# Elyptos/VolumetricRaytracer

Measured on AMD Instinct MI355X. Metric: Mrays/sec at 1080p, 256^3 SDF volume, higher is better.
Workload: dtype f32

## Files before the change

### volumetricraytracer_amd/csrc/vrt_device.h

```cpp
#pragma once
#include <stdint.h>

namespace vrt {

constexpr int kBrickCells = 4;
constexpr int kBrickSamples = 5;
constexpr int kBrickFloats = 128;
constexpr int kPathCube = 8;
constexpr int kPathBrick16 = 9;
constexpr int kPathCube16 = 10;
constexpr int kPathCells16 = 11;
constexpr int kNibWindow = 16;
constexpr int kTile = 8;
constexpr int kBlockThreads = 256;
constexpr int kMaxBvhNodes = 2 * 64 - 1;
constexpr int kStatWords = 7;
constexpr int kStatRecord = 8;
constexpr int kDiagRecord = 8;
constexpr int kMaxBlocks = 1 << 20;
#ifndef VRT_MAX_BLOCK_FRAMES
#define VRT_MAX_BLOCK_FRAMES 48
#endif
constexpr int kMaxBlockFrames = VRT_MAX_BLOCK_FRAMES;
constexpr int kMaxLaunchFrames = 256;

constexpr int kMapSupertile = 0;
constexpr int kMapBand = 1;
constexpr int kMapLinear = 2;

inline int grid_blocks(int tiles_x, int tiles_y, int tile_map) {
    if (tile_map != kMapSupertile) return tiles_x * tiles_y;
    const int st = ((tiles_x + 3) / 4) * ((tiles_y + 3) / 4);
    return ((st + 7) / 8) * 8 * 16;
}

struct DVolume {
    const float* dense;
    const void* bricks;
    const void* cells;
    int32_t N;
    int32_t nb;
    float extent;
    float inv_cell;
    float density_scale;
    float step_max;
    float tint[3];
    float roughness;
    float metallic;
    float k;
    float cell;
    int32_t format;
    const uint8_t* skip;
    const uint32_t* nib;
    const uint8_t* tex_px[3];
    int32_t tex_w[3], tex_h[3];
    float tex_scale[2];
// ... 133 lines not shown
```

### volumetricraytracer_amd/csrc/vrt_kernels.hip

```cpp
#include <hip/hip_runtime.h>
#include <math.h>
#include <stdlib.h>
#include "vrt_device.h"
#include "vrt_launch.h"
#include "voxelize_core.h"
#include "brush_core.h"

namespace vrt {

struct F3 {
    float x, y, z;
};
__device__ __forceinline__ F3 f3(float x, float y, float z) { return F3{x, y, z}; }
__device__ __forceinline__ F3 operator+(F3 a, F3 b) { return f3(a.x + b.x, a.y + b.y, a.z + b.z); }
__device__ __forceinline__ F3 operator-(F3 a, F3 b) { return f3(a.x - b.x, a.y - b.y, a.z - b.z); }
__device__ __forceinline__ F3 operator*(F3 a, float s) { return f3(a.x * s, a.y * s, a.z * s); }
__device__ __forceinline__ float dot3(F3 a, F3 b) { return (a.x * b.x + a.y * b.y) + a.z * b.z; }
__device__ __forceinline__ F3 normalize3(F3 a) {
    float inv = 1.0f / sqrtf(dot3(a, a));
    return a * inv;
}
__device__ __forceinline__ float maxf_(float a, float b) { return a > b ? a : b; }
__device__ __forceinline__ float minf_(float a, float b) { return a < b ? a : b; }
__device__ __forceinline__ F3 mul33(const float* m, F3 v) {
// ... 694 lines not shown
        return march_cube<NORMAL, PATH == kPathCube16>(F, I, Vd, o, d, t_cur, t_hit, n_world, steps, ex);
    } else {
    constexpr int DP = data_path<PATH>();
    const VolRef V = load_vol<DP>(Vd);
    RaySeg R;
    if constexpr (DIR_SHADOW) {
        if (!setup_shadow_ray(F, I, V, o, t_cur, t_base, R)) return false;
    } else {
        if (!setup_ray(F, I, V, o, d, t_cur, t_base, R)) return false;
    }
    MarchState st;
    st.t = st.t_prev = R.t0;
    st.s_prev = st.s_hit = 0.0f;
    st.i = 0;
    st.hit = false;
    st.chk = __builtin_inff();
    st.c = Cell{0, 0, 0, 0.0f, 0.0f, 0.0f};
    march_lane<DP, DIAG, MULTI>(F, V, R, st, F.max_steps, steps, dg);
    if (!st.hit) {
        if (F.max_steps > 0 && st.i >= F.max_steps && !(st.t > R.t_end)) ex += kExhaustedOne;
        return false;
    }
    float t = st.t;
    Cell c = st.c;
    if (st.s_hit < 0.0f && st.i > 0) t = refine_hit<DP>(V, R, st.t_prev, st.s_prev, t, st.s_hit, c, steps);
    else if (NORMAL != 0 && F.polish > 0 && st.i > 0) t = polish_hit<DP>(F, V, R, t, st.s_hit, st.t_prev, st.s_prev, F.polish, c, steps);
    t_hit = t;
    if constexpr (NORMAL == 1) n_world = hit_normal<DP, false, REF>(I, V, R, c, st.i, REF && F.zero_outside != 0);
    if constexpr (NORMAL == 2) n_world = hit_normal<DP, true, REF>(I, V, R, c, st.i, REF && F.zero_outside != 0);
    return true;
    }
}

template <int PATH, bool SINGLE, bool DIAG = false, int NORMAL = 1, bool REF = false>
__device__ __forceinline__ bool trace_closest(const DFrame& F, F3 o, F3 d, float t_max, float t_base, float& t_best,
                                              int& inst_best, F3& n_best, unsigned& steps, unsigned& ex, DiagAcc* dg = nullptr) {
    if constexpr (SINGLE) {
        float t;
        F3 n;
        if (march_instance<PATH, NORMAL, DIAG, false, REF>(F, F.inst, F.vol0, o, d, t_max, t_base, t, n, steps, ex, dg)) {
            t_best = t;
            inst_best = 0;
            n_best = n;
            return true;
        }
        return false;
    } else {
        bool any = false;
        float best = t_max;
        int ni = 0;
        while (ni < F.n_nodes) {
            ni = __builtin_amdgcn_readfirstlane(ni);
            const DBvhNode nd = F.nodes[ni];
            const bool in = slab_box(o, d, nd, best);
            if (__ballot(in) == 0ull) {
                ni = nd.right;
                continue;
            }
            if (nd.left < 0) {
                const int ii = -nd.left - 1;
                const DInstance* I = F.inst + ii;
                if (in) {
                    float t;
                    F3 n;
                    constexpr bool kCube = PATH == kPathCube || PATH == kPathCube16;
                    if (march_instance<PATH, NORMAL, DIAG, false, REF, true>(F, I, F.vols + I->slot, o, d, kCube ? best : t_max, t_base, t, n, steps, ex, dg)) {
                        if (!any || t < best || (t == best && ii < inst_best)) {
                            any = true;
                            best = t;
                            t_best = t;
                            inst_best = ii;
                            n_best = n;
                        }
                    }
                }
                ni = nd.right;
            } else {
                ni = ni + 1;
            }
        }
        return any;
    }
}

template <int PATH, bool SINGLE, bool DIAG = false, bool DIR_SHADOW = false>
__device__ __forceinline__ bool trace_any(const DFrame& F, F3 o, F3 d, float t_max, float t_base, unsigned& steps, unsigned& ex,
                                          DiagAcc* dg = nullptr) {
    float t;
    F3 n;
    if constexpr (SINGLE) {
        return march_instance<PATH, 0, DIAG, DIR_SHADOW>(F, F.inst, F.vol0, o, d, t_max, t_base, t, n, steps, ex, dg);
    } else {
        bool found = false;
        int ni = 0;
        while (ni < F.n_nodes) {
            if (__ballot(!found) == 0ull) break;
            ni = __builtin_amdgcn_readfirstlane(ni);
            const DBvhNode nd = F.nodes[ni];
            const bool in = !found && slab_box(o, d, nd, t_max);
            if (__ballot(in) == 0ull) {
                ni = nd.right;
                continue;
            }
            if (nd.left < 0) {
                const DInstance* I = F.inst + (-nd.left - 1);
                if (in && march_instance<PATH, 0, DIAG, DIR_SHADOW, false, true>(F, I, F.vols + I->slot, o, d, t_max, t_base, t, n, steps, ex, dg)) found = true;
                ni = nd.right;
            } else {
                ni = ni + 1;
            }
        }
        return found;
    }
}

__device__ __forceinline__ unsigned env_fetch(const uint8_t* __restrict__ env, int S, F3 dir) {
    if (env == nullptr) return 0u;
    float vx = dir.x, vy = dir.z, vz = dir.y;
    float ax = fabsf(vx), ay = fabsf(vy), az = fabsf(vz);
    int face;
    float sc, tc, ma;
    if (ax >= ay && ax >= az) {
        ma = ax;
        if (vx >= 0.0f) { face = 0; sc = -vz; tc = -vy; }
        else            { face = 1; sc = vz;  tc = -vy; }
    } else if (ay >= az) {
        ma = ay;
        if (vy >= 0.0f) { face = 2; sc = vx; tc = vz; }
        else            { face = 3; sc = vx; tc = -vz; }
    } else {
        ma = az;
        if (vz >= 0.0f) { face = 4; sc = vx;  tc = -vy; }
        else            { face = 5; sc = -vx; tc = -vy; }
    }
    const float inv_ma = 1.0f / ma;
    float u = (sc * inv_ma + 1.0f) * 0.5f;
    float v = (tc * inv_ma + 1.0f) * 0.5f;
    int ix = (int)floorf(u * (float)S);
    int iy = (int)floorf(v * (float)S);
// ... 22 lines not shown
    float m = maxf_(-wdoth + 1.0f, 0.0f);
    float m2 = m * m;
    float m5 = (m2 * m2) * m;
    F3 Fr = f3(f0.x + (-f0.x + 1.0f) * m5, f0.y + (-f0.y + 1.0f) * m5, f0.z + (-f0.z + 1.0f) * m5);
    float dwo = maxf_(dot3(n, wo), 0.0f);
    float dwi = maxf_(dot3(n, wi), 0.0f);
    float G = (dwo * fast_rcp(dwo * (1.0f - k) + k)) * (dwi * fast_rcp(dwi * (1.0f - k) + k));
    float dg = (D * G) * fast_rcp(maxf_((4.0f * dwo) * dwi, 0.0001f));
    F3 cook = f3(dg * Fr.x, dg * Fr.y, dg * Fr.z);
    float km = 1.0f - metal;
    F3 kd = f3((1.0f - Fr.x) * km, (1.0f - Fr.y) * km, (1.0f - Fr.z) * km);
    return f3((albedo.x * INV_PI_REF) * kd.x + cook.x * Fr.x, (albedo.y * INV_PI_REF) * kd.y + cook.y * Fr.y,
              (albedo.z * INV_PI_REF) * kd.z + cook.z * Fr.z);
}

__device__ __forceinline__ F3 radiance(F3 Li, F3 wi, F3 wo, F3 n, F3 albedo, float rough, float metal, float k) {
    const F3 brdf = brdf_eval(wi, wo, n, albedo, rough, metal, k);
    const float ndwi = dot3(n, wi);
    return f3((brdf.x * Li.x) * ndwi, (brdf.y * Li.y) * ndwi, (brdf.z * Li.z) * ndwi);
}

__device__ __forceinline__ float tonemap(float c) {
    c = c > 0.0f ? c : 0.0f;
    c = c * fast_rcp(c + 1.0f);
    return fast_pow(c, 1.0f / 2.2f);
}

__device__ __forceinline__ unsigned wave_sum(unsigned v) {
#pragma unroll
    for (int o = 32; o > 0; o >>= 1) v += __shfl_xor(v, o);
    return v;
}

__device__ __forceinline__ void tile_of_block(const DFrame& F, int b, int nblk, int& tile_x, int& tile_y) {
    if (F.tile_map == kMapSupertile) {
        const int rot = (int)blockIdx.y;
        const int xcd = (b + rot) & 7, q = b >> 3;
        const int st = (q >> 4) * 8 + xcd;
        const int within = q & 15;
        const int st_x = (F.tiles_x + 3) >> 2;
        tile_x = (st % st_x) * 4 + (within & 3);
        tile_y = (st / st_x) * 4 + (within >> 2);
    } else if (F.tile_map == kMapBand) {
        const int xcd = b & 7, q = b >> 3;
        const int per = nblk >> 3, rem = nblk & 7;
        const int L = (xcd < rem) ? xcd * (per + 1) + q : rem * (per + 1) + (xcd - rem) * per + q;
        tile_x = L % F.tiles_x;
        tile_y = L / F.tiles_x;
    } else {
        tile_x = b % F.tiles_x;
        tile_y = b / F.tiles_x;
    }
}

constexpr int kMarchThreads = 64;
constexpr int kMarchGridMul = 4;
__device__ __forceinline__ void block_and_wave(int& b, int& wave) {
    const int raw = (int)blockIdx.x, xcd = raw & 7, q = raw >> 3;
    wave = q & 3;
    b = ((q >> 2) << 3) | xcd;
}

__device__ __forceinline__ void pixel_of_lane(int tile_x, int tile_y, int wave, int lane, int& px, int& pyl) {
    px = tile_x * 16 + (wave & 1) * 8 + (lane & 7);
    pyl = tile_y * 16 + (wave >> 1) * 8 + (lane >> 3);
}

__device__ __forceinline__ bool wave_can_reach(const DCam& C, bool valid, int px, int py) {
    const int x0 = (int)(C.cull_lo & 0xffffu), y0 = (int)(C.cull_lo >> 16), x1 = (int)(C.cull_hi & 0xffffu), y1 = (int)(C.cull_hi >> 16);
    const bool inside = px >= x0 && px <= x1 && py >= y0 && py <= y1;
    return __ballot(valid && inside) != 0ull;
}

__device__ __forceinline__ DCam load_cam(const DBlock& B, int frame) {
    typedef unsigned u16v __attribute__((ext_vector_type(16)));
    u16v w;
    if (B.f.cams != nullptr) w = *reinterpret_cast<const u16v __attribute__((address_space(4)))*>((const __attribute__((address_space(4))) DCam*)B.f.cams + frame);
    else w = *reinterpret_cast<const u16v*>(&B.cam[frame]);
    DCam C;
    C.cam_o[0] = __uint_as_float(w[0]); C.cam_o[1] = __uint_as_float(w[1]); C.cam_o[2] = __uint_as_float(w[2]);
    C.r0[0] = __uint_as_float(w[3]); C.r0[1] = __uint_as_float(w[4]); C.r0[2] = __uint_as_float(w[5]);
    C.r1[0] = __uint_as_float(w[6]); C.r1[1] = __uint_as_float(w[7]); C.r1[2] = __uint_as_float(w[8]);
    C.r2[0] = __uint_as_float(w[9]); C.r2[1] = __uint_as_float(w[10]); C.r2[2] = __uint_as_float(w[11]);
    C.cx = __uint_as_float(w[12]); C.cy = __uint_as_float(w[13]);
    C.cull_lo = w[14]; C.cull_hi = w[15];
    return C;
}

template <bool DYN>
__device__ __forceinline__ const DFrame& frame_view(const DBlock& B, int frame, DFrame& Fd) {
    if constexpr (!DYN) {
        (void)frame;
        (void)Fd;
        return B.f;
    } else {
        typedef unsigned u16v __attribute__((ext_vector_type(16)));
        Fd = B.f;
        const char* sec = static_cast<const char*>(B.f.dyn) + (size_t)(unsigned)frame * kDynStride;
        const u16v w = *reinterpret_cast<const u16v __attribute__((address_space(4)))*>((const __attribute__((address_space(4))) char*)sec);
        Fd.light_dir[0] = __uint_as_float(w[0]);
        Fd.light_dir[1] = __uint_as_float(w[1]);
        Fd.light_dir[2] = __uint_as_float(w[2]);
        Fd.light_strength = __uint_as_float(w[3]);
        Fd.n_inst = (int)w[4];
        Fd.n_nodes = (int)w[5];
        Fd.n_point = (int)w[6];
        Fd.n_spot = (int)w[7];
        Fd.vol0 = B.f.vols + (int)w[8];
        Fd.inst = reinterpret_cast<const DInstance*>(sec + kDynInstOff);
        Fd.nodes = reinterpret_cast<const DBvhNode*>(sec + kDynNodesOff);
        Fd.point = reinterpret_cast<const DPointLight*>(sec + kDynPointOff);
        Fd.spot = reinterpret_cast<const DSpotLight*>(sec + kDynSpotOff);
        return Fd;
    }
}

__device__ __forceinline__ void camera_ray(const DFrame& F, const DCam& C, int px, int py, F3& o, F3& d) {
    float sx = (((float)px + 0.5f) * F.inv_w) * 2.0f - 1.0f;
    float sy = (((float)py + 0.5f) * F.inv_h) * 2.0f - 1.0f;
// ... 202 lines not shown
    return q;
}
__device__ __forceinline__ F3 rotate_vector(F3 v, Q4 r) {
    Q4 rc = {-r.x, -r.y, -r.z, r.w};
    Q4 vq = {v.x, v.y, v.z, 0.0f};
    const Q4 t = qmul(r, qmul(vq, rc));
    return f3(t.x, t.y, t.z);
}

template <bool CONST_ONLY = false>
__device__ __forceinline__ void textured_surface(const DVolume* __restrict__ V, const DInstance* __restrict__ I, F3 hit_world,
                                                 F3& albedo, F3& n, float& rough, float& metal) {
    const F3 op = mul33(I->w2o, f3(hit_world.x - I->pos[0], hit_world.y - I->pos[1], hit_world.z - I->pos[2]));
    const F3 no = mul33(I->w2o, n);
    const F3 an = f3(fabsf(no.x), fabsf(no.y), fabsf(no.z));
    const float sum = (an.x + an.y) + an.z;
    const F3 blend = f3(an.x / sum, an.y / sum, an.z / sum);
    if (V->tex_px[0] != nullptr) {
        const F3 t = tri_sample<CONST_ONLY>(V, 0, op, blend, false);
        albedo = f3(albedo.x * t.x, albedo.y * t.y, albedo.z * t.z);
    }
    if (V->tex_px[2] != nullptr) {
        const F3 t = tri_sample<CONST_ONLY>(V, 2, op, blend, false);
        rough = minf_(maxf_(V->roughness_raw * t.x, 0.0f), 1.0f);
        metal = minf_(maxf_(V->metallic_raw * t.y, 0.0f), 1.0f);
    }
    if (V->tex_px[1] != nullptr) {
        F3 t = tri_sample<CONST_ONLY>(V, 1, op, blend, true);
        t = normalize3(t);
        n = mul33(I->o2w, rotate_vector(f3(t.z, t.x, t.y), quat_from_x(no)));
    }
}

template <int PATH, bool SINGLE, bool DIAG, bool DYN = false,
          bool REF = false >
#ifndef VRT_BVH_WAVES
#define VRT_BVH_WAVES 7
#endif
__global__ __launch_bounds__(kMarchThreads) __attribute__((amdgpu_waves_per_eu((!SINGLE && !DIAG && PATH != VRT_PATH_DENSE) ? VRT_BVH_WAVES : (REF && SINGLE) ? 8 : 1))) void march_kernel(const DBlock B) {
    unsigned long long t_start = 0;
    if constexpr (DIAG) t_start = __builtin_amdgcn_s_memrealtime();
    const int frame = (int)blockIdx.y;
    DFrame Fd;
    const DFrame& F = frame_view<DYN>(B, frame, Fd);
    const DCam C = load_cam(B, frame);
    int b, wave;
    block_and_wave(b, wave);
    int tile_x, tile_y;
    tile_of_block(F, b, (int)gridDim.x / kMarchGridMul, tile_x, tile_y);
    const int lane = (int)threadIdx.x & 63;
    int px, pyl;
    pixel_of_lane(tile_x, tile_y, wave, lane, px, pyl);
    const int py = frame_row(F, pyl);
    const bool valid = tile_x < F.tiles_x && tile_y < F.tiles_y && px < F.width && pyl < F.rows && py < F.height;

    Counters k;
    DiagAcc dg;
    const bool reach = wave_can_reach(C, valid, px, py);

    if (valid) {
        F3 o, d;
        camera_ray(F, C, px, py, o, d);
        k.n_primary = 1;
        float t_hit = 0.0f;
        int inst = 0;
        F3 n = f3(0.0f, 0.0f, 0.0f);
        F3 color;
        const unsigned sky = env_fetch(F.env, F.env_size, d);
        if (reach && trace_closest<PATH, SINGLE, DIAG, 2, REF>(F, o, d, 10000.0f, 0.0f, t_hit, inst, n, k.s_primary, k.n_hits, &dg)) {
            k.n_hits += 1;
            bool shadowed = false;
            const F3 ld = f3(F.light_dir[0], F.light_dir[1], F.light_dir[2]);
            if constexpr (REF) {
                const DVolume* V = SINGLE ? F.vol0 : F.vols + F.inst[inst].slot;
                F3 albedo = f3(V->tint[0], V->tint[1], V->tint[2]);
                float rough = V->roughness, metal = V->metallic;
                if (F.textured) {
                    const F3 hp = f3(__builtin_fmaf(d.x, t_hit, o.x), __builtin_fmaf(d.y, t_hit, o.y), __builtin_fmaf(d.z, t_hit, o.z));
                    textured_surface<true>(V, SINGLE ? F.inst : F.inst + inst, hp, albedo, n, rough, metal);
                }
                if (F.shadow && !F.unlit && dot3(n, ld) > 0.0f) {
                    k.n_shadow = 1;
                    const float vs = F.view_vec ? camera_len(F, C, px, py) : 1.0f;
                    shadowed = trace_any<PATH, SINGLE, DIAG, true>(F, shadow_origin(F, o, d, t_hit, vs), ld, 5000.0f, t_hit, k.s_shadow, k.n_hits, &dg);
                }
                const float vs = F.view_vec ? camera_len(F, C, px, py) : 1.0f;
                color = shade_hit_surface(F, V, d, vs, n, albedo, rough, metal, shadowed);
            } else {
            if (F.shadow && !F.unlit && dot3(n, ld) > 0.0f) {
                k.n_shadow = 1;
                shadowed = trace_any<PATH, SINGLE, DIAG, true>(F, shadow_origin(F, o, d, t_hit), ld, 5000.0f, t_hit, k.s_shadow, k.n_hits, &dg);
            }
            color = shade_hit(F, SINGLE ? F.vol0 : F.vols + F.inst[inst].slot, d, n, shadowed);
            }
        } else {
            color = env_decode(sky);
        }
        store_pixel(F, frame, (unsigned)pyl * (unsigned)F.width + (unsigned)px, color);
    }
    write_records<DIAG, true>(F, frame, b, wave, lane, k, dg, t_start);
}

constexpr int kMaxDepth = 3;

#ifndef VRT_FULL_WAVES
#define VRT_FULL_WAVES 1
#endif
__device__ __forceinline__ size_t pass_record(const DFrame& F, int frame, int b, int wave, int lane) {
    return (size_t)(unsigned)frame * F.rec_stride + (size_t)(((unsigned)b * 4u + (unsigned)wave) * 64u + (unsigned)lane);
}
__device__ __forceinline__ size_t pass_wave(const DFrame& F, int frame, int b, int wave) {
    return ((size_t)(unsigned)frame * F.rec_stride >> 6) + (size_t)((unsigned)b * 4u + (unsigned)wave);
}
constexpr unsigned kShadowBitDir = 1u << 16, kShadowBitPoint = 2u << 16, kShadowBitSpot = 64u << 16;

__device__ __forceinline__ F3 direct_light_from_bits(const DFrame& F, F3 so, F3 wo, F3 n, F3 albedo, float rough, float metal, float kk,
                                                     bool shadows, bool bounce, unsigned bits) {
    F3 sum = f3(0.0f, 0.0f, 0.0f);
    {
        const F3 ld = f3(F.light_dir[0], F.light_dir[1], F.light_dir[2]);
        const bool lone_backfacing = F.n_point == 0 && F.n_spot == 0 && !bounce && !(dot3(n, ld) > 0.0f);
        const bool sh = shadows && !lone_backfacing && (bits & kShadowBitDir) != 0u;
        if (!sh) sum = sum + radiance(f3(F.light_strength, F.light_strength, F.light_strength), ld, wo, n, albedo, rough, metal, kk);
    }
    for (int i = 0; i < F.n_point; i++) {
        const DPointLight L = F.point[i];
        const F3 dl = f3(L.pos[0] - so.x, L.pos[1] - so.y, L.pos[2] - so.z);
        const float dist = sqrtf(dot3(dl, dl));
        const float inten = L.intensity / ((1.0f + L.att_linear * dist) + (L.att_exp * dist) * dist);
        if (inten > 0.005f) {
            const F3 ld = dl * (1.0f / dist);
            const bool sh = shadows && (bits & (kShadowBitPoint << i)) != 0u;
            if (!sh) sum = sum + radiance(f3(L.color[0] * inten, L.color[1] * inten, L.color[2] * inten), ld, wo, n, albedo, rough, metal, kk);
// ... 6 lines not shown
        const F3 sd = f3(-dl.x, -dl.y, -dl.z) * (1.0f / dist);
        const float cs = dot3(f3(L.fwd[0], L.fwd[1], L.fwd[2]), sd);
        float inten = 0.0f;
        if (cs >= 0.0f && cs > L.cos_angle) {
            const float delta = (cs - L.cos_angle) / (L.cos_falloff - L.cos_angle);
            const float base = L.intensity * minf_(delta, 1.0f);
            inten = base / ((1.0f + L.att_linear * dist) + (L.att_exp * dist) * dist);
        }
        if (inten > 0.01f) {
            const F3 ld = dl * (1.0f / dist);
            const bool sh = shadows && (bits & (kShadowBitSpot << i)) != 0u;
            if (!sh) sum = sum + radiance(f3(L.color[0] * inten, L.color[1] * inten, L.color[2] * inten), ld, wo, n, albedo, rough, metal, kk);
        }
    }
    return sum;
}

template <int PATH, bool SINGLE, bool SHADE_PASS = false, bool DYN = false>
__global__ __launch_bounds__(kMarchThreads) __attribute__((amdgpu_waves_per_eu(VRT_FULL_WAVES))) void march_kernel_full(const DBlock B) {
    const int frame = (int)blockIdx.y;
    DFrame Fd;
    const DFrame& F = frame_view<DYN>(B, frame, Fd);
    int b, wave;
    block_and_wave(b, wave);
    const int lane = (int)threadIdx.x & 63;
    bool rec_hit = false;
    if constexpr (SHADE_PASS) {
        const unsigned long long m = F.hit_mask[pass_wave(F, frame, b, wave)];
        if (m == 0ull) return;
        rec_hit = ((m >> lane) & 1ull) != 0ull;
    }
    const DCam C = load_cam(B, frame);
    int tile_x, tile_y;
    tile_of_block(F, b, (int)gridDim.x / kMarchGridMul, tile_x, tile_y);
    int px, pyl;
    pixel_of_lane(tile_x, tile_y, wave, lane, px, pyl);
    const int py = frame_row(F, pyl);
    const bool valid = SHADE_PASS ? rec_hit : (tile_x < F.tiles_x && tile_y < F.tiles_y && px < F.width && pyl < F.rows && py < F.height);

    Counters k;
    DiagAcc dg;
    const bool reach = SHADE_PASS ? true : wave_can_reach(C, valid, px, py);
    if (valid) {
        F3 o, d;
        camera_ray(F, C, px, py, o, d);
        if constexpr (!SHADE_PASS) k.n_primary = 1;
        F3 direct[kMaxDepth - 1], brdf[kMaxDepth - 1];
        float ndwi[kMaxDepth - 1], fade[kMaxDepth - 1];
        int pending = 0;
        float t_base = 0.0f;
        F3 color = f3(0.0f, 0.0f, 0.0f);
        unsigned shadow_bits = 0u;
#pragma unroll 1
        for (int level = 1; level <= kMaxDepth; level++) {
            float t_hit = 0.0f;
            int inst = 0;
            F3 n = f3(0.0f, 0.0f, 0.0f);
            if (SHADE_PASS && level == 1) {
                const size_t r = pass_record(F, frame, b, wave, lane);
                const HitRecord h = F.hit_rec[r];
                const unsigned aux = F.hit_aux[r];
                t_hit = h.t;
                n = f3(h.nx, h.ny, h.nz);
                inst = (int)(aux & 0xffffu);
                shadow_bits = aux;
            } else {
                if ((level == 1 && !reach) || !trace_closest<PATH, SINGLE, false, 2, true>(F, o, d, 10000.0f, t_base, t_hit, inst, n, k.s_primary, k.n_hits)) {
// ... 88 lines not shown
                color = f3(0.0f, 0.0f, 0.0f);
                continue;
            }
            color = sum;
            break;
        }
        for (int j = pending - 1; j >= 0; j--) {
            const F3 rc = f3(maxf_(0.0f, color.x + (0.0f - color.x) * fade[j]), maxf_(0.0f, color.y + (0.0f - color.y) * fade[j]),
                             maxf_(0.0f, color.z + (0.0f - color.z) * fade[j]));
            const F3 r = f3((brdf[j].x * rc.x) * ndwi[j], (brdf[j].y * rc.y) * ndwi[j], (brdf[j].z * rc.z) * ndwi[j]);
            color = direct[j] + r;
        }
        store_pixel(F, frame, (unsigned)pyl * (unsigned)F.width + (unsigned)px, color);
    }
    write_records<false, false, SHADE_PASS>(F, frame, b, wave, lane, k, dg, 0ull);
}

#ifndef VRT_PRIMARY_PASS_WAVES
#define VRT_PRIMARY_PASS_WAVES 7
#endif
#ifndef VRT_SHADOW_PASS_WAVES
#define VRT_SHADOW_PASS_WAVES 7
#endif
template <int PATH, bool SINGLE, bool DYN = false>
__global__ __launch_bounds__(kMarchThreads) __attribute__((amdgpu_waves_per_eu((!SINGLE && PATH != VRT_PATH_DENSE) ? VRT_PRIMARY_PASS_WAVES : 1)))
void primary_pass_kernel(const DBlock B) {
    const int frame = (int)blockIdx.y;
    DFrame Fd;
    const DFrame& F = frame_view<DYN>(B, frame, Fd);
    const DCam C = load_cam(B, frame);
    int b, wave;
    block_and_wave(b, wave);
    int tile_x, tile_y;
    tile_of_block(F, b, (int)gridDim.x / kMarchGridMul, tile_x, tile_y);
    const int lane = (int)threadIdx.x & 63;
    int px, pyl;
    pixel_of_lane(tile_x, tile_y, wave, lane, px, pyl);
    const int py = frame_row(F, pyl);
    const bool valid = tile_x < F.tiles_x && tile_y < F.tiles_y && px < F.width && pyl < F.rows && py < F.height;

    Counters k;
    DiagAcc dg;
    const bool reach = wave_can_reach(C, valid, px, py);
    bool hit = false;
    if (valid) {
        F3 o, d;
        camera_ray(F, C, px, py, o, d);
        k.n_primary = 1;
        float t_hit = 0.0f;
        int inst = 0;
        F3 n = f3(0.0f, 0.0f, 0.0f);
        const unsigned sky = env_fetch(F.env, F.env_size, d);
        if (reach && trace_closest<PATH, SINGLE, false, 2, true>(F, o, d, 10000.0f, 0.0f, t_hit, inst, n, k.s_primary, k.n_hits)) {
            k.n_hits += 1;
            hit = true;
            const size_t r = pass_record(F, frame, b, wave, lane);
            F.hit_rec[r] = HitRecord{n.x, n.y, n.z, t_hit};
            F.hit_aux[r] = (unsigned)inst;
        } else {
            store_pixel(F, frame, (unsigned)pyl * (unsigned)F.width + (unsigned)px, env_decode(sky));
        }
    }
    const unsigned long long m = __ballot(hit);
    if (lane == 0) F.hit_mask[pass_wave(F, frame, b, wave)] = m;
    write_records<false, true>(F, frame, b, wave, lane, k, dg, 0ull);
}

template <int PATH, bool SINGLE, bool DYN = false>
__global__ __launch_bounds__(kMarchThreads) __attribute__((amdgpu_waves_per_eu(SINGLE ? 8 : VRT_SHADOW_PASS_WAVES))) void light_pass_kernel(const DBlock B) {
    const int frame = (int)blockIdx.y;
    DFrame Fd;
    const DFrame& F = frame_view<DYN>(B, frame, Fd);
    int b, wave;
    block_and_wave(b, wave);
    const int lane = (int)threadIdx.x & 63;
    const unsigned long long m = F.hit_mask[pass_wave(F, frame, b, wave)];
    if (m == 0ull) return;
    const DCam C = load_cam(B, frame);
    int tile_x, tile_y;
    tile_of_block(F, b, (int)gridDim.x / kMarchGridMul, tile_x, tile_y);
    int px, pyl;
    pixel_of_lane(tile_x, tile_y, wave, lane, px, pyl);
    const int py = frame_row(F, pyl);
    Counters k;
    DiagAcc dg;
    bool bounces = false;
    if (((m >> lane) & 1ull) != 0ull) {
        F3 o, d;
        camera_ray(F, C, px, py, o, d);
        const size_t r = pass_record(F, frame, b, wave, lane);
        unsigned bits = 0u;
        if (F.shadow && !F.unlit) {
            const HitRecord h = F.hit_rec[r];
            const F3 so = shadow_origin(F, o, d, h.t, F.view_vec ? camera_len(F, C, px, py) : 1.0f);
            const float tb = 0.0f + h.t;
            const F3 sun = f3(F.light_dir[0], F.light_dir[1], F.light_dir[2]);
            bool cast_sun = true;
            if (F.n_point == 0 && F.n_spot == 0) {
                const int inst = (int)F.hit_aux[r];
                const DVolume* V = SINGLE ? F.vol0 : F.vols + F.inst[inst].slot;
                F3 n = f3(h.nx, h.ny, h.nz);
                F3 albedo = f3(V->tint[0], V->tint[1], V->tint[2]);
                float rough = V->roughness, metal = V->metallic;
                if (F.textured) {
                    const F3 hp = f3(__builtin_fmaf(d.x, h.t, o.x), __builtin_fmaf(d.y, h.t, o.y), __builtin_fmaf(d.z, h.t, o.z));
                    textured_surface(V, SINGLE ? F.inst : F.inst + inst, hp, albedo, n, rough, metal);
                }
                const bool bounce = rough < 0.3f && 1 <= F.max_bounces;
                cast_sun = bounce || dot3(n, sun) > 0.0f;
            }
            if (cast_sun) {
                k.n_shadow++;
                if (trace_any<PATH, SINGLE, false, true>(F, so, sun, 5000.0f, tb, k.s_shadow, k.n_hits)) bits |= kShadowBitDir;
// ... 181 lines not shown
    st.hit = false;
    st.chk = __builtin_inff();
    st.c = Cell{0, 0, 0, 0.0f, 0.0f, 0.0f};
    const int max_steps = F.max_steps;
    const int head = max_steps < kHeadSteps ? max_steps : kHeadSteps;
    if (act) march_lane<VRT_PATH_BRICK, false>(F, V, R, st, head, steps, nullptr);
    const bool cont = act && !st.hit && st.i < max_steps && !(st.t > R.t_end);
    if (__ballot(cont) != 0ull) march_tail_lds(F, V, R, cont, st, slots, tags, lane, steps);
    if (!st.hit) {
        if (act && max_steps > 0 && st.i >= max_steps && !(st.t > R.t_end)) ex += kExhaustedOne;
        return false;
    }
    float t = st.t;
    Cell c = st.c;
    if (st.s_hit < 0.0f && st.i > 0) t = refine_hit<VRT_PATH_BRICK>(V, R, st.t_prev, st.s_prev, t, st.s_hit, c, steps);
    else if (CLOSEST && F.polish > 0 && st.i > 0) t = polish_hit<VRT_PATH_BRICK>(F, V, R, t, st.s_hit, st.t_prev, st.s_prev, F.polish, c, steps);
    t_hit = t;
    c_hit = c;
    iter_hit = st.i;
    return true;
}

template <bool DIAG>
__global__ __launch_bounds__(kBlockThreads) void march_kernel_coop(const DBlock B) {
    __shared__ float s_slots[4][kLdsSlots * kBrickFloats];
    __shared__ unsigned s_tags[4][kLdsSlots];
    unsigned long long t_start = 0;
    if constexpr (DIAG) t_start = __builtin_amdgcn_s_memrealtime();
    const DFrame& F = B.f;
    const int frame = (int)blockIdx.y;
    const DCam C = load_cam(B, frame);
    const int b = (int)blockIdx.x;
    int tile_x, tile_y;
    tile_of_block(F, b, (int)gridDim.x, tile_x, tile_y);
    const int wave = (int)threadIdx.x >> 6;
    const int lane = (int)threadIdx.x & 63;
    int px, pyl;
    pixel_of_lane(tile_x, tile_y, wave, lane, px, pyl);
    const int py = frame_row(F, pyl);
    const bool valid = tile_x < F.tiles_x && tile_y < F.tiles_y && px < F.width && pyl < F.rows && py < F.height;

    float* slots = s_slots[wave];
    unsigned* tags = s_tags[wave];
    if (lane < kLdsSlots) tags[lane] = kTagInvalid;
    __builtin_amdgcn_fence(__ATOMIC_RELEASE, "wavefront");
    __builtin_amdgcn_wave_barrier();

    Counters k;
    DiagAcc dg;
    const DInstance* I = F.inst;
    const DVolume* Vd = F.vol0;
    const VolRef V = load_vol<VRT_PATH_BRICK>(Vd);

    F3 o = f3(0.0f, 0.0f, 0.0f), d = f3(1.0f, 0.0f, 0.0f);
    RaySeg R = {};
    bool act = false;
    const bool reach = wave_can_reach(C, valid, px, py);
    if (valid) {
        camera_ray(F, C, px, py, o, d);
        k.n_primary = 1;
        if (reach) act = setup_ray(F, I, V, o, d, 10000.0f, 0.0f, R);
    }
    float t_hit = 0.0f;
    Cell c_hit = {0, 0, 0, 0.0f, 0.0f, 0.0f};
    int iter_hit = 0;
    const bool hit = march_hybrid<true>(F, V, R, act, slots, tags, lane, t_hit, c_hit, iter_hit, k.s_primary, k.n_hits);

// ... 474 lines not shown
hipError_t launch_gather_ceiling(const void* pool, unsigned n_bricks, int format, bool coherent, int iters, float* out, int blocks, hipStream_t stream) {
    const dim3 g((unsigned)blocks), t(256);
    const char* p = static_cast<const char*>(pool);
    if (format == VRT_FORMAT_TEXEL16) {
        if (coherent) hipLaunchKernelGGL((gather_ceiling_kernel<kPathBrick16, true>), g, t, 0, stream, p, n_bricks - 1, iters, out);
        else hipLaunchKernelGGL((gather_ceiling_kernel<kPathBrick16, false>), g, t, 0, stream, p, n_bricks - 1, iters, out);
    } else {
        if (coherent) hipLaunchKernelGGL((gather_ceiling_kernel<VRT_PATH_BRICK, true>), g, t, 0, stream, p, n_bricks - 1, iters, out);
        else hipLaunchKernelGGL((gather_ceiling_kernel<VRT_PATH_BRICK, false>), g, t, 0, stream, p, n_bricks - 1, iters, out);
    }
    return hipGetLastError();
}


static bool needs_ref_kernel(const DFrame& F) { return F.textured != 0 || F.view_vec != 0 || F.zero_outside != 0; }

template <int PATH, bool SINGLE>
static hipError_t launch_t(const DBlock& B, hipStream_t stream) {
    const DFrame& F = B.f;
    const int grid = grid_blocks(F.tiles_x, F.tiles_y, F.tile_map);
    if (grid <= 0) return hipSuccess;
    if (F.diag)
        hipLaunchKernelGGL((march_kernel<PATH, SINGLE, true>), dim3((unsigned)(grid * kMarchGridMul), (unsigned)F.n_frames), dim3(kMarchThreads), 0, stream, B);
    else
        hipLaunchKernelGGL((march_kernel<PATH, SINGLE, false>), dim3((unsigned)(grid * kMarchGridMul), (unsigned)F.n_frames), dim3(kMarchThreads), 0, stream, B);
    return hipGetLastError();
}

template <int PATH, bool SINGLE>
static hipError_t launch_nodiag_t(const DBlock& B, hipStream_t stream) {
    const DFrame& F = B.f;
    const int grid = grid_blocks(F.tiles_x, F.tiles_y, F.tile_map);
    if (grid <= 0) return hipSuccess;
    const dim3 g((unsigned)(grid * kMarchGridMul), (unsigned)F.n_frames), t(kMarchThreads);
    if (needs_ref_kernel(F)) {
        if (F.dyn != nullptr) hipLaunchKernelGGL((march_kernel<PATH, SINGLE, false, true, true>), g, t, 0, stream, B);
        else hipLaunchKernelGGL((march_kernel<PATH, SINGLE, false, false, true>), g, t, 0, stream, B);
    } else if (F.dyn != nullptr) {
        hipLaunchKernelGGL((march_kernel<PATH, SINGLE, false, true>), g, t, 0, stream, B);
    } else {
        hipLaunchKernelGGL((march_kernel<PATH, SINGLE, false>), g, t, 0, stream, B);
    }
    return hipGetLastError();
}

static hipError_t launch_coop(const DBlock& B, hipStream_t stream) {
    const DFrame& F = B.f;
    const int grid = grid_blocks(F.tiles_x, F.tiles_y, F.tile_map);
    if (grid <= 0) return hipSuccess;
    if (F.diag)
        hipLaunchKernelGGL((march_kernel_coop<true>), dim3((unsigned)grid, (unsigned)F.n_frames), dim3(kBlockThreads), 0, stream, B);
    else
        hipLaunchKernelGGL((march_kernel_coop<false>), dim3((unsigned)grid, (unsigned)F.n_frames), dim3(kBlockThreads), 0, stream, B);
    return hipGetLastError();
}

template <int PATH, bool SINGLE>
static hipError_t launch_full_t(const DBlock& B, hipStream_t stream) {
    const DFrame& F = B.f;
    const int grid = grid_blocks(F.tiles_x, F.tiles_y, F.tile_map);
    if (grid <= 0) return hipSuccess;
    const dim3 g((unsigned)(grid * kMarchGridMul), (unsigned)F.n_frames), t(kMarchThreads);
    if (F.dyn != nullptr) {
        if (F.hit_rec != nullptr) {
            hipLaunchKernelGGL((primary_pass_kernel<PATH, SINGLE, true>), g, t, 0, stream, B);
            hipLaunchKernelGGL((light_pass_kernel<PATH, SINGLE, true>), g, t, 0, stream, B);
            if (F.may_bounce) hipLaunchKernelGGL((march_kernel_full<PATH, false, true, true>), g, t, 0, stream, B);
// ... 287 lines not shown
```

Before: 64930.

## Process multiple frames per wave in single-instance march kernel

Single-instance, non-diag march kernels now have each wave render several consecutive frames (default two) for the same pixel tile, so the grid's y dimension shrinks by that factor. Waves whose tile misses every frame's cull box write sky pixels for all frames in a fast path. Instance and volume pointers are reinterpreted as constant-address-space views so their loads can go through scalar memory. The aim is to amortize per-block setup and reuse scalar data across frames, at the cost of less parallelism and longer-running waves. The diag launch path still sizes the grid per frame.

```diff
diff --git a/volumetricraytracer_amd/csrc/vrt_device.h b/volumetricraytracer_amd/csrc/vrt_device.h
--- a/volumetricraytracer_amd/csrc/vrt_device.h
+++ b/volumetricraytracer_amd/csrc/vrt_device.h
@@ -22,6 +22,12 @@
 #define VRT_MAX_BLOCK_FRAMES 48
 #endif
 constexpr int kMaxBlockFrames = VRT_MAX_BLOCK_FRAMES;
+#ifndef VRT_FRAMES_PER_WAVE
+#define VRT_FRAMES_PER_WAVE 2
+#endif
+constexpr int kFramesPerWave = VRT_FRAMES_PER_WAVE;
+static_assert(kFramesPerWave >= 1 && kFramesPerWave <= 8, "frames per wave");
+constexpr int frames_per_wave(bool single, bool diag) { return (diag || !single) ? 1 : kFramesPerWave; }
 constexpr int kMaxLaunchFrames = 256;
 
 constexpr int kMapSupertile = 0;
diff --git a/volumetricraytracer_amd/csrc/vrt_kernels.hip b/volumetricraytracer_amd/csrc/vrt_kernels.hip
--- a/volumetricraytracer_amd/csrc/vrt_kernels.hip
+++ b/volumetricraytracer_amd/csrc/vrt_kernels.hip
@@ -750,13 +750,26 @@
     }
 }
 
-template <int PATH, bool SINGLE, bool DIAG = false, int NORMAL = 1, bool REF = false>
+template <typename T>
+__device__ __forceinline__ const T* constant_view(const T* p) {
+    const __attribute__((address_space(4))) T* c = (const __attribute__((address_space(4))) T*)p;
+    asm("" : "+s"(c));
+    return (const T*)c;
+}
+template <bool CV, typename T>
+__device__ __forceinline__ const T* cv(const T* p) {
+    if constexpr (CV) return constant_view(p);
+    else return p;
+}
+
+template <int PATH, bool SINGLE, bool DIAG = false, int NORMAL = 1, bool REF = false,
+          bool CV = false >
 __device__ __forceinline__ bool trace_closest(const DFrame& F, F3 o, F3 d, float t_max, float t_base, float& t_best,
                                               int& inst_best, F3& n_best, unsigned& steps, unsigned& ex, DiagAcc* dg = nullptr) {
     if constexpr (SINGLE) {
         float t;
         F3 n;
-        if (march_instance<PATH, NORMAL, DIAG, false, REF>(F, F.inst, F.vol0, o, d, t_max, t_base, t, n, steps, ex, dg)) {
+        if (march_instance<PATH, NORMAL, DIAG, false, REF>(F, cv<CV>(F.inst), cv<CV>(F.vol0), o, d, t_max, t_base, t, n, steps, ex, dg)) {
             t_best = t;
             inst_best = 0;
             n_best = n;
@@ -767,9 +780,12 @@
         bool any = false;
         float best = t_max;
         int ni = 0;
+        const DBvhNode* const nodes = cv<CV>(F.nodes);
+        const DInstance* const insts = cv<CV>(F.inst);
+        const DVolume* const vols = cv<CV>(F.vols);
         while (ni < F.n_nodes) {
             ni = __builtin_amdgcn_readfirstlane(ni);
-            const DBvhNode nd = F.nodes[ni];
+            const DBvhNode nd = nodes[ni];
             const bool in = slab_box(o, d, nd, best);
             if (__ballot(in) == 0ull) {
                 ni = nd.right;
@@ -777,12 +793,12 @@
             }
             if (nd.left < 0) {
                 const int ii = -nd.left - 1;
-                const DInstance* I = F.inst + ii;
+                const DInstance* I = insts + ii;
                 if (in) {
                     float t;
                     F3 n;
                     constexpr bool kCube = PATH == kPathCube || PATH == kPathCube16;
-                    if (march_instance<PATH, NORMAL, DIAG, false, REF, true>(F, I, F.vols + I->slot, o, d, kCube ? best : t_max, t_base, t, n, steps, ex, dg)) {
+                    if (march_instance<PATH, NORMAL, DIAG, false, REF, true>(F, I, vols + I->slot, o, d, kCube ? best : t_max, t_base, t, n, steps, ex, dg)) {
                         if (!any || t < best || (t == best && ii < inst_best)) {
                             any = true;
                             best = t;
@@ -801,28 +817,31 @@
     }
 }
 
-template <int PATH, bool SINGLE, bool DIAG = false, bool DIR_SHADOW = false>
+template <int PATH, bool SINGLE, bool DIAG = false, bool DIR_SHADOW = false, bool CV = false>
 __device__ __forceinline__ bool trace_any(const DFrame& F, F3 o, F3 d, float t_max, float t_base, unsigned& steps, unsigned& ex,
                                           DiagAcc* dg = nullptr) {
     float t;
     F3 n;
     if constexpr (SINGLE) {
-        return march_instance<PATH, 0, DIAG, DIR_SHADOW>(F, F.inst, F.vol0, o, d, t_max, t_base, t, n, steps, ex, dg);
+        return march_instance<PATH, 0, DIAG, DIR_SHADOW>(F, cv<CV>(F.inst), cv<CV>(F.vol0), o, d, t_max, t_base, t, n, steps, ex, dg);
     } else {
         bool found = false;
         int ni = 0;
+        const DBvhNode* const nodes = cv<CV>(F.nodes);
+        const DInstance* const insts = cv<CV>(F.inst);
+        const DVolume* const vols = cv<CV>(F.vols);
         while (ni < F.n_nodes) {
             if (__ballot(!found) == 0ull) break;
             ni = __builtin_amdgcn_readfirstlane(ni);
-            const DBvhNode nd = F.nodes[ni];
+            const DBvhNode nd = nodes[ni];
             const bool in = !found && slab_box(o, d, nd, t_max);
             if (__ballot(in) == 0ull) {
                 ni = nd.right;
                 continue;
             }
             if (nd.left < 0) {
-                const DInstance* I = F.inst + (-nd.left - 1);
-                if (in && march_instance<PATH, 0, DIAG, DIR_SHADOW, false, true>(F, I, F.vols + I->slot, o, d, t_max, t_base, t, n, steps, ex, dg)) found = true;
+                const DInstance* I = insts + (-nd.left - 1);
+                if (in && march_instance<PATH, 0, DIAG, DIR_SHADOW, false, true>(F, I, vols + I->slot, o, d, t_max, t_base, t, n, steps, ex, dg)) found = true;
                 ni = nd.right;
             } else {
                 ni = ni + 1;
@@ -911,9 +930,8 @@
     return v;
 }
 
-__device__ __forceinline__ void tile_of_block(const DFrame& F, int b, int nblk, int& tile_x, int& tile_y) {
+__device__ __forceinline__ void tile_of_block(const DFrame& F, int b, int nblk, int rot , int& tile_x, int& tile_y) {
     if (F.tile_map == kMapSupertile) {
-        const int rot = (int)blockIdx.y;
         const int xcd = (b + rot) & 7, q = b >> 3;
         const int st = (q >> 4) * 8 + xcd;
         const int within = q & 15;
@@ -945,11 +963,12 @@
     pyl = tile_y * 16 + (wave >> 1) * 8 + (lane >> 3);
 }
 
-__device__ __forceinline__ bool wave_can_reach(const DCam& C, bool valid, int px, int py) {
-    const int x0 = (int)(C.cull_lo & 0xffffu), y0 = (int)(C.cull_lo >> 16), x1 = (int)(C.cull_hi & 0xffffu), y1 = (int)(C.cull_hi >> 16);
+__device__ __forceinline__ bool wave_can_reach(unsigned cull_lo, unsigned cull_hi, bool valid, int px, int py) {
+    const int x0 = (int)(cull_lo & 0xffffu), y0 = (int)(cull_lo >> 16), x1 = (int)(cull_hi & 0xffffu), y1 = (int)(cull_hi >> 16);
     const bool inside = px >= x0 && px <= x1 && py >= y0 && py <= y1;
     return __ballot(valid && inside) != 0ull;
 }
+__device__ __forceinline__ bool wave_can_reach(const DCam& C, bool valid, int px, int py) { return wave_can_reach(C.cull_lo, C.cull_hi, valid, px, py); }
 
 __device__ __forceinline__ DCam load_cam(const DBlock& B, int frame) {
     typedef unsigned u16v __attribute__((ext_vector_type(16)));
@@ -964,6 +983,14 @@
     C.cx = __uint_as_float(w[12]); C.cy = __uint_as_float(w[13]);
     C.cull_lo = w[14]; C.cull_hi = w[15];
     return C;
+}
+__device__ __forceinline__ void load_cull(const DBlock& B, int frame, unsigned& cull_lo, unsigned& cull_hi) {
+    typedef unsigned u2v __attribute__((ext_vector_type(2)));
+    u2v w;
+    if (B.f.cams != nullptr) w = *reinterpret_cast<const u2v __attribute__((address_space(4)))*>(&((const __attribute__((address_space(4))) DCam*)B.f.cams + frame)->cull_lo);
+    else w = *reinterpret_cast<const u2v*>(&B.cam[frame].cull_lo);
+    cull_lo = w[0];
+    cull_hi = w[1];
 }
 
 template <bool DYN>
@@ -1232,25 +1259,16 @@
     }
 }
 
-template <int PATH, bool SINGLE, bool DIAG, bool DYN = false,
-          bool REF = false >
 #ifndef VRT_BVH_WAVES
 #define VRT_BVH_WAVES 7
 #endif
-__global__ __launch_bounds__(kMarchThreads) __attribute__((amdgpu_waves_per_eu((!SINGLE && !DIAG && PATH != VRT_PATH_DENSE) ? VRT_BVH_WAVES : (REF && SINGLE) ? 8 : 1))) void march_kernel(const DBlock B) {
-    unsigned long long t_start = 0;
-    if constexpr (DIAG) t_start = __builtin_amdgcn_s_memrealtime();
-    const int frame = (int)blockIdx.y;
+template <int PATH, bool SINGLE, bool DIAG, bool DYN,
+          bool REF >
+__device__ __forceinline__ void march_frame(const DBlock& B, int frame, const DCam& C, int b, int wave, int lane, int tile_x, int tile_y, int px, int pyl,
+                                            unsigned long long t_start) {
     DFrame Fd;
     const DFrame& F = frame_view<DYN>(B, frame, Fd);
-    const DCam C = load_cam(B, frame);
-    int b, wave;
-    block_and_wave(b, wave);
-    int tile_x, tile_y;
-    tile_of_block(F, b, (int)gridDim.x / kMarchGridMul, tile_x, tile_y);
-    const int lane = (int)threadIdx.x & 63;
-    int px, pyl;
-    pixel_of_lane(tile_x, tile_y, wave, lane, px, pyl);
+    constexpr bool CV = frames_per_wave(SINGLE, DIAG) > 1;
     const int py = frame_row(F, pyl);
     const bool valid = tile_x < F.tiles_x && tile_y < F.tiles_y && px < F.width && pyl < F.rows && py < F.height;
 
@@ -1267,31 +1285,31 @@
         F3 n = f3(0.0f, 0.0f, 0.0f);
         F3 color;
         const unsigned sky = env_fetch(F.env, F.env_size, d);
-        if (reach && trace_closest<PATH, SINGLE, DIAG, 2, REF>(F, o, d, 10000.0f, 0.0f, t_hit, inst, n, k.s_primary, k.n_hits, &dg)) {
+        if (reach && trace_closest<PATH, SINGLE, DIAG, 2, REF, CV>(F, o, d, 10000.0f, 0.0f, t_hit, inst, n, k.s_primary, k.n_hits, &dg)) {
             k.n_hits += 1;
             bool shadowed = false;
             const F3 ld = f3(F.light_dir[0], F.light_dir[1], F.light_dir[2]);
             if constexpr (REF) {
-                const DVolume* V = SINGLE ? F.vol0 : F.vols + F.inst[inst].slot;
+                const DVolume* V = SINGLE ? cv<CV>(F.vol0) : cv<CV>(F.vols) + cv<CV>(F.inst)[inst].slot;
                 F3 albedo = f3(V->tint[0], V->tint[1], V->tint[2]);
                 float rough = V->roughness, metal = V->metallic;
                 if (F.textured) {
                     const F3 hp = f3(__builtin_fmaf(d.x, t_hit, o.x), __builtin_fmaf(d.y, t_hit, o.y), __builtin_fmaf(d.z, t_hit, o.z));
-                    textured_surface<true>(V, SINGLE ? F.inst : F.inst + inst, hp, albedo, n, rough, metal);
+                    textured_surface<true>(V, SINGLE ? cv<CV>(F.inst) : cv<CV>(F.inst) + inst, hp, albedo, n, rough, metal);
                 }
                 if (F.shadow && !F.unlit && dot3(n, ld) > 0.0f) {
                     k.n_shadow = 1;
                     const float vs = F.view_vec ? camera_len(F, C, px, py) : 1.0f;
-                    shadowed = trace_any<PATH, SINGLE, DIAG, true>(F, shadow_origin(F, o, d, t_hit, vs), ld, 5000.0f, t_hit, k.s_shadow, k.n_hits, &dg);
+                    shadowed = trace_any<PATH, SINGLE, DIAG, true, CV>(F, shadow_origin(F, o, d, t_hit, vs), ld, 5000.0f, t_hit, k.s_shadow, k.n_hits, &dg);
                 }
                 const float vs = F.view_vec ? camera_len(F, C, px, py) : 1.0f;
                 color = shade_hit_surface(F, V, d, vs, n, albedo, rough, metal, shadowed);
             } else {
             if (F.shadow && !F.unlit && dot3(n, ld) > 0.0f) {
                 k.n_shadow = 1;
-                shadowed = trace_any<PATH, SINGLE, DIAG, true>(F, shadow_origin(F, o, d, t_hit), ld, 5000.0f, t_hit, k.s_shadow, k.n_hits, &dg);
-            }
-            color = shade_hit(F, SINGLE ? F.vol0 : F.vols + F.inst[inst].slot, d, n, shadowed);
+                shadowed = trace_any<PATH, SINGLE, DIAG, true, CV>(F, shadow_origin(F, o, d, t_hit), ld, 5000.0f, t_hit, k.s_shadow, k.n_hits, &dg);
+            }
+            color = shade_hit(F, SINGLE ? cv<CV>(F.vol0) : cv<CV>(F.vols) + cv<CV>(F.inst)[inst].slot, d, n, shadowed);
             }
         } else {
             color = env_decode(sky);
@@ -1299,6 +1317,80 @@
         store_pixel(F, frame, (unsigned)pyl * (unsigned)F.width + (unsigned)px, color);
     }
     write_records<DIAG, true>(F, frame, b, wave, lane, k, dg, t_start);
+}
+
+template <int PATH, bool SINGLE, bool DIAG, bool DYN, bool REF>
+__device__ __forceinline__ void march_group(const DBlock& B) {
+    unsigned long long t_start = 0;
+    if constexpr (DIAG) t_start = __builtin_amdgcn_s_memrealtime();
+    constexpr int R = frames_per_wave(SINGLE, DIAG);
+    const int group = (int)blockIdx.y, f0 = group * R;
+    const DCam C0 = load_cam(B, f0);
+    int b, wave;
+    block_and_wave(b, wave);
+    int tile_x, tile_y;
+    tile_of_block(B.f, b, (int)gridDim.x / kMarchGridMul, group, tile_x, tile_y);
+    const int lane = (int)threadIdx.x & 63;
+    int px, pyl;
+    pixel_of_lane(tile_x, tile_y, wave, lane, px, pyl);
+    if constexpr (R == 1) {
+        march_frame<PATH, SINGLE, DIAG, DYN, REF>(B, f0, C0, b, wave, lane, tile_x, tile_y, px, pyl, t_start);
+    } else {
+        const int left = B.f.n_frames - f0, nf = left < R ? left : R;
+        const DFrame& F = B.f;
+        const int py = frame_row(F, pyl);
+        const bool valid = tile_x < F.tiles_x && tile_y < F.tiles_y && px < F.width && pyl < F.rows && py < F.height;
+        bool any_reach = false;
+#pragma unroll
+        for (int r = 0; r < R; ++r) {
+            if (r < nf) {
+                unsigned lo = C0.cull_lo, hi = C0.cull_hi;
+                if (r > 0) load_cull(B, f0 + r, lo, hi);
+                any_reach |= wave_can_reach(lo, hi, valid, px, py);
+            }
+        }
+        if (!any_reach) {
+            const unsigned pix = (unsigned)pyl * (unsigned)F.width + (unsigned)px;
+            unsigned sky[R];
+#pragma unroll
+            for (int r = 0; r < R; ++r) {
+                sky[r] = 0u;
+                if (r < nf && valid) {
+                    const DCam C = r == 0 ? C0 : load_cam(B, f0 + r);
+                    F3 o, d;
+                    camera_ray(F, C, px, py, o, d);
+                    sky[r] = env_fetch(F.env, F.env_size, d);
+                }
+            }
+#pragma unroll
+            for (int r = 0; r < R; ++r) {
+                if (r < nf) {
+                    Counters k;
+                    if (valid) {
+                        k.n_primary = 1;
+                        store_pixel(F, f0 + r, pix, env_decode(sky[r]));
+                    }
+                    write_records<false, true>(F, f0 + r, b, wave, lane, k, DiagAcc(), 0ull);
+                }
+            }
+            return;
+        }
+        int px_r = px, pyl_r = pyl;
+#pragma unroll
+        for (int r = 0; r < R; ++r) {
+            if (r >= nf) break;
+            const __attribute__((address_space(4))) void* ka = (const __attribute__((address_space(4))) void*)__builtin_amdgcn_kernarg_segment_ptr();
+            asm("" : "+s"(ka) : "s"(r));
+            const DBlock& Br = *reinterpret_cast<const DBlock*>((const void*)ka);
+            march_frame<PATH, SINGLE, DIAG, DYN, REF>(Br, f0 + r, r == 0 ? C0 : load_cam(Br, f0 + r), b, wave, lane, tile_x, tile_y, px_r, pyl_r, t_start);
+            asm("" : "+v"(px_r), "+v"(pyl_r) : "s"(r));
+        }
+    }
+}
+
+template <int PATH, bool SINGLE, bool DIAG, bool DYN = false, bool REF = false >
+__global__ __launch_bounds__(kMarchThreads) __attribute__((amdgpu_waves_per_eu((!SINGLE && !DIAG && PATH != VRT_PATH_DENSE) ? VRT_BVH_WAVES : (REF && SINGLE) ? 8 : 1))) void march_kernel(const DBlock B) {
+    march_group<PATH, SINGLE, DIAG, DYN, REF>(B);
 }
 
 constexpr int kMaxDepth = 3;
@@ -1371,7 +1463,7 @@
     }
     const DCam C = load_cam(B, frame);
     int tile_x, tile_y;
-    tile_of_block(F, b, (int)gridDim.x / kMarchGridMul, tile_x, tile_y);
+    tile_of_block(F, b, (int)gridDim.x / kMarchGridMul, (int)blockIdx.y, tile_x, tile_y);
     int px, pyl;
     pixel_of_lane(tile_x, tile_y, wave, lane, px, pyl);
     const int py = frame_row(F, pyl);
@@ -1526,7 +1618,7 @@
     int b, wave;
     block_and_wave(b, wave);
     int tile_x, tile_y;
-    tile_of_block(F, b, (int)gridDim.x / kMarchGridMul, tile_x, tile_y);
+    tile_of_block(F, b, (int)gridDim.x / kMarchGridMul, (int)blockIdx.y, tile_x, tile_y);
     const int lane = (int)threadIdx.x & 63;
     int px, pyl;
     pixel_of_lane(tile_x, tile_y, wave, lane, px, pyl);
@@ -1572,7 +1664,7 @@
     if (m == 0ull) return;
     const DCam C = load_cam(B, frame);
     int tile_x, tile_y;
-    tile_of_block(F, b, (int)gridDim.x / kMarchGridMul, tile_x, tile_y);
+    tile_of_block(F, b, (int)gridDim.x / kMarchGridMul, (int)blockIdx.y, tile_x, tile_y);
     int px, pyl;
     pixel_of_lane(tile_x, tile_y, wave, lane, px, pyl);
     const int py = frame_row(F, pyl);
@@ -1820,7 +1912,7 @@
     const DCam C = load_cam(B, frame);
     const int b = (int)blockIdx.x;
     int tile_x, tile_y;
-    tile_of_block(F, b, (int)gridDim.x, tile_x, tile_y);
+    tile_of_block(F, b, (int)gridDim.x, (int)blockIdx.y, tile_x, tile_y);
     const int wave = (int)threadIdx.x >> 6;
     const int lane = (int)threadIdx.x & 63;
     int px, pyl;
@@ -2361,7 +2453,8 @@
     const DFrame& F = B.f;
     const int grid = grid_blocks(F.tiles_x, F.tiles_y, F.tile_map);
     if (grid <= 0) return hipSuccess;
-    const dim3 g((unsigned)(grid * kMarchGridMul), (unsigned)F.n_frames), t(kMarchThreads);
+    constexpr int R = frames_per_wave(SINGLE, false);
+    const dim3 g((unsigned)(grid * kMarchGridMul), (unsigned)((F.n_frames + R - 1) / R)), t(kMarchThreads);
     if (needs_ref_kernel(F)) {
         if (F.dyn != nullptr) hipLaunchKernelGGL((march_kernel<PATH, SINGLE, false, true, true>), g, t, 0, stream, B);
         else hipLaunchKernelGGL((march_kernel<PATH, SINGLE, false, false, true>), g, t, 0, stream, B);
```

Result: no change. 64450 (-0.7%).
